# troyvvgroup/quemb

Hardware: AMD Instinct MI355X
Metric: fragment CCSD iters/sec (full BE sweep over synthetic n_occ=20 n_virt=200 fragments); corr-E error vs oracle in parity_max_abs_err_Eh / parity_n220_abs_err_Eh (higher is better)
Workload: dtype f64

## Files before the change

include/qemb_hip_ops.h:

```cpp
#ifndef QEMB_HIP_OPS_H
#define QEMB_HIP_OPS_H
#include "qemb_hip.h"
#ifdef __cplusplus
extern "C" {
#endif

#define QEMB_TIMER_LADDER 0
#define QEMB_TIMER_RINGS 1
#define QEMB_TIMER_ITER 2
#define QEMB_TIMER_AO2MO 3
#define QEMB_TIMER_SCF 4
#define QEMB_TIMER_GEMM_ANY 5
#define QEMB_TIMER_SCHMIDT 6
#define QEMB_TIMER_DF 7
int qemb_timer_begin(int slot);
int qemb_timer_end(int slot);
int qemb_timer_read(int slot, double* total_ms, int64_t* count);
int qemb_timer_reset(int slot);
int qemb_alloc_stats(long long* n_driver_allocs, long long* n_driver_frees, double* ms_in_driver_calls, double* gb_allocated, int reset);
int qemb_gemm_flop_count(double* flops, int reset);
int qemb_tape_cache_counters(int64_t* reused, int64_t* recorded, int reset);
int qemb_ctx_timer_read(int ctx, int slot, double* total_ms, int64_t* count, int reset);
int qemb_timer_live_events(int slot);

// ... 24 lines not shown
int qemb_op_dot(int64_t n, const double* x, const double* y, double* out_dev);
int qemb_op_absmax(int64_t n, const double* x, double* out_dev);
int qemb_op_gemv_rows(int64_t rows, int64_t cols, const double* T, int64_t ldt, const double* x, double* y,
                      double alpha, double beta);
int qemb_op_gemv_rows_batched(int64_t rows, int64_t cols, int64_t nbatch, const double* T, int64_t ldt, int64_t strideT,
                              const double* x, int64_t stridex, double* y, double alpha, double beta);
int qemb_op_contract_mid(int64_t outer, int64_t mid, int64_t inner, const double* T, const double* x,
                         double* Y, int64_t ldy, double alpha, double beta);
int qemb_op_unpack_s4(int64_t n, const double* s4, double* s1);
int qemb_op_pack_s4(int64_t n, const double* s1, double* s4);
int qemb_op_unpack_s8_to_s4(int64_t n, const double* s8, double* s4);
int qemb_op_mirror_lower(int64_t n, double* A, int64_t lda);
int qemb_op_k_from_pairs(int64_t n, const double* H, const double* D, double* K);
int qemb_op_jk_from_packed(int64_t n, const double* S4, const double* D, const double* Dp, double* Jp, double* K);
int qemb_op_pack_pm_cols(int64_t rows, int64_t v, const double* in, double* Op, int64_t ldp, double* Om, int64_t ldm);
int qemb_op_scatter_pm_rows(int64_t o, int64_t ncols, const double* Xp, const double* Xm, double* out);
int qemb_op_pack_w_pm(int64_t o, const double* W, double* Ap, int64_t lda_p, double* Am, int64_t lda_m);
int qemb_op_ladder_scatter_pm2(int64_t o, int64_t v, const double* Rp, int64_t ldp, const double* Rm, int64_t ldm, const double* Hp, const double* Hm,
                               int assign, double* t2);
int qemb_op_lincomb2(int64_t n, double a, const double* x, double b, const double* y, double beta, double* out);
int qemb_op_small_k_update(int64_t batch, int64_t M, int64_t N, int64_t K, double alpha, const double* A, int64_t sA, const double* B, int64_t sB, double* C, int64_t sC);
int qemb_op_ccsd_ph_layouts(int64_t o, int64_t v, const double* t2, const double* t1, double* T, double* Tp, double* S, double* Ut, double* Tpt, double* Th);
int qemb_op_ccsd_y_traces(int64_t o, int64_t v, const double* ZC, const double* ZB, double* Y);
int qemb_op_copy4_two(const int64_t dim[4], const double* in, const int64_t si[4], double* out, const int64_t so[4], double alpha, double beta, const double* base,
                      double* out2, const double* in2, double c2a, double c2b);
int qemb_op_scatter_pm_rows_add(int64_t o, int64_t ncols, const double* Xp, const double* Xm, double* out, const double* add);
int qemb_op_ccsd_y_traces_add(int64_t o, int64_t v, const double* ZC, const double* ZB, double* Y, const double* add);
int qemb_op_pack_w_pm_sum(int64_t o, const double* Wt, const double* X, const double* At, double* Ap, int64_t lda_p, double* Am, int64_t lda_m);
int qemb_op_ccsd_t1_small(int64_t o, int64_t v, const double* t1, const double* Lvv, const double* Loo, const double* Fov, double* t1n);
int qemb_op_ccsd_t1_assemble(int64_t o, int64_t v, const double* t1, const double* Lvv, const double* Loo, const double* Fov, const double* S, const double* Lph1,
                             const double* PA, int SA, int64_t strideA, const double* PB, int SB, int64_t strideB, double* t1n);
int qemb_op_gemv_rows_two(int64_t rows1, int64_t cols1, const double* T1, int64_t ld1, const double* x1, double* y1, double a1, double b1,
                          int64_t rows2, int64_t cols2, const double* T2, int64_t ld2, const double* x2, double* y2, double a2, double b2);
int qemb_op_ccsd_y_traces_slabs(int64_t o, int64_t v, const double* ZC, const double* ZB, double* Y, const double* add, int S, int64_t stride, double scale);
int qemb_op_gemv_rows2(int64_t rows, int64_t cols, const double* T1, int64_t ld1, const double* x1, const double* T2, int64_t ld2, const double* x2, double* y, double alpha, double beta);
int qemb_op_ccsd_finish_t2_rings(int64_t o, int64_t v, double* t2n, const double* U, const double* OV, const double* RS, const double* M, const double* eo, const double* ev, double* t1n);
int qemb_op_diis_push(int64_t n, const double* trial, const double* prev, double* e, double* xcopy, int m, const double* const* ys, int self, double* row_dev, double* row_host);
int qemb_op_ccsd_extrapolate_energy(int64_t o, int64_t v, int nterms, const double* coef, const double* const* xs, double* amp, const double* L, double* tau, double* e_host);
int qemb_op_gather_rows(int64_t nrows, int64_t len, const int64_t* idx_dev, const double* src, int64_t ld, double* dst);
int qemb_op_scale_rows(int64_t nrows, int64_t len, double* x, const double* s);
int qemb_op_pack_pair_rows(int64_t n, int64_t ncols, const double* in, double* out);
int qemb_op_unpack_tril_pair_rows(int64_t nr, int64_t n, const double* in, double* full);
int qemb_op_extract_pf(int64_t n, const double* Mp, int64_t p0, int64_t q0, int64_t r0, int64_t s0, int64_t sp, int64_t sq,
                       int64_t sr, int64_t ss, double* out);
int qemb_op_extract_pf_t(int64_t n, const double* T, int64_t x0, int64_t r0, int64_t s0, int64_t c0, int64_t sx, int64_t sr,
                         int64_t ss, int64_t sc, double* out);
// ... 40 lines not shown
```

quemb_amd/_lib.py:

```python

from __future__ import annotations

import ctypes as C
import os
from pathlib import Path

import numpy as np

_HERE = Path(__file__).resolve().parent
LIB_PATH = _HERE / "libqemb_hip.so"

c_dp = C.POINTER(C.c_double)
c_i64 = C.c_int64
c_vp = C.c_void_p


QEMB_ERR_ARG, QEMB_ERR_ALLOC, QEMB_ERR_DEVICE, QEMB_ERR_NOCONV, QEMB_ERR_NUMERIC, QEMB_ERR_UNSUPPORTED = -1, -2, -3, -4, -5, -6


class QembError(RuntimeError):

    def __init__(self, msg="", status=None):
        super().__init__(msg)
        self.status = status
# ... 58 lines not shown
    f("qemb_op_rdm2_add_nc", I, L, P, D, P)
    f("qemb_op_rdm2_symmetrize", I, L, P, P)
    f("qemb_op_rdm2_eri_dot", I, L, I, P, P, C.POINTER(D))
    f("qemb_op_absmax", I, L, P, P)
    f("qemb_op_gemv_rows", I, L, L, P, L, P, P, D, D)
    f("qemb_op_gemv_rows_batched", I, L, L, L, P, L, L, P, L, P, D, D)
    f("qemb_op_contract_mid", I, L, L, L, P, P, P, L, D, D)
    f("qemb_op_unpack_s4", I, L, P, P)
    f("qemb_op_pack_s4", I, L, P, P)
    f("qemb_op_unpack_s8_to_s4", I, L, P, P)
    f("qemb_op_unpack_tril_rows", I, L, L, P, P)
    f("qemb_op_pack_pair_rows", I, L, L, P, P)
    f("qemb_op_mirror_lower", I, L, P, L)
    f("qemb_op_k_from_pairs", I, L, P, P, P)
    f("qemb_op_jk_from_packed", I, L, P, P, P, P, P)
    f("qemb_op_pack_pm_cols", I, L, L, P, P, L, P, L)
    f("qemb_op_scatter_pm_rows", I, L, L, P, P, P)
    f("qemb_op_pack_w_pm", I, L, P, P, L, P, L)
    f("qemb_op_ladder_scatter_pm2", I, L, L, P, L, P, L, P, P, I, P)
    f("qemb_op_lincomb2", I, L, D, P, D, P, D, P)
    f("qemb_op_small_k_update", I, L, L, L, L, D, P, L, P, L, P, L)
    f("qemb_op_ccsd_ph_layouts", I, L, L, P, P, P, P, P, P, P, P)
    f("qemb_op_ccsd_y_traces", I, L, L, P, P, P)
    f("qemb_op_copy4_two", I, C.POINTER(L), P, C.POINTER(L), P, C.POINTER(L), D, D, P, P, P, D, D)
    f("qemb_op_scatter_pm_rows_add", I, L, L, P, P, P, P)
    f("qemb_op_ccsd_y_traces_add", I, L, L, P, P, P, P)
    f("qemb_op_pack_w_pm_sum", I, L, P, P, P, P, L, P, L)
    f("qemb_op_ccsd_t1_small", I, L, L, P, P, P, P, P)
    f("qemb_op_gemv_rows2", I, L, L, P, L, P, P, L, P, P, D, D)
    f("qemb_op_ccsd_t1_assemble", I, L, L, P, P, P, P, P, P, P, I, L, P, I, L, P)
    f("qemb_op_gemv_rows_two", I, L, L, P, L, P, P, D, D, L, L, P, L, P, P, D, D)
    f("qemb_op_ccsd_y_traces_slabs", I, L, L, P, P, P, P, I, L, D)
    f("qemb_op_ccsd_finish_t2_rings", I, L, L, P, P, P, P, P, P, P, P)
    f("qemb_op_diis_push", I, L, P, P, P, P, I, P, I, P, P)
    f("qemb_op_ccsd_extrapolate_energy", I, L, L, I, P, P, P, P, P, P)
    f("qemb_op_gather_rows", I, L, L, P, P, L, P)
    f("qemb_op_scale_rows", I, L, L, P, P)
    f("qemb_ctx_count", I, I)
    f("qemb_ctx_bind", I, I)
    f("qemb_ctx_partition", I, I)
    f("qemb_ctx_timer_read", I, I, I, C.POINTER(C.c_double), C.POINTER(c_i64), I)
    f("qemb_gemm_flop_count", I, C.POINTER(C.c_double), I)
    f("qemb_tape_cache_counters", I, C.POINTER(L), C.POINTER(L), I)
    f("qemb_alloc_stats", I, C.POINTER(C.c_longlong), C.POINTER(C.c_longlong), C.POINTER(C.c_double), C.POINTER(C.c_double), I)
    f("qemb_op_unpack_tril_pair_rows", I, L, L, P, P)
    f("qemb_op_extract_pf", I, L, P, L, L, L, L, L, L, L, L, P)
# ... 195 lines not shown
```

quemb_amd/csrc/api.cpp:

```cpp
#include <cstring>
#include <cstdlib>
#include <vector>
#include <execinfo.h>
#include <signal.h>
#include <unistd.h>
#include "../../include/qemb_hip_ops.h"
#include "dev_ops.h"
#include "ccsd.h"
#include "fragment.h"
#include "ao2mo.h"
#include "kdf.h"
#include "int3c.h"
#include "int4c.h"
#include <mutex>
#include <set>

using namespace qemb;
namespace qemb {
int dev_mfma_f64_peak(int iters, int blocks_per_cu, double* tflops);
int schmidt_eigh(const double* lmo, int N, int nmo, int nocc, const int64_t* frag, int n_f, double thr, double* TA_out,
                 int ld_out, int* n_b_out, int* sweeps_out);
int schmidt_subspace(const double* lmo, int N, int nmo, int nocc, const int64_t* frag, int n_f, double thr, double* TA_out,
                     int ld_out, int* n_b_out, int* sweeps_out);
int schmidt_svd(const double* rdm, int N, const int64_t* frag_in, int n_f, double thr, double* TA_out, int ld_out, int* n_b_out,
// ... 125 lines not shown
  tape_cache_counters(&a, &b, reset);
  if (reused) *reused = a;
  if (recorded) *recorded = b;
  return QEMB_OK;
}
int qemb_alloc_stats(long long* n, long long* nfree, double* ms, double* gb, int reset) { return dev_alloc_stats(n, nfree, ms, gb, reset); }
int qemb_ctx_timer_read(int ctx, int slot, double* total_ms, int64_t* count, int reset) { return dev_ctx_timer_read(ctx, slot, total_ms, count, reset); }
int qemb_op_k_from_pairs(int64_t n, const double* H, const double* D, double* K) { return dev_k_from_pairs(n, H, D, K); }
int qemb_op_jk_from_packed(int64_t n, const double* S4, const double* D, const double* Dp, double* Jp, double* K) { return dev_jk_from_packed(n, S4, D, Dp, Jp, K); }
int qemb_op_pack_pm_cols(int64_t rows, int64_t v, const double* in, double* Op, int64_t ldp, double* Om, int64_t ldm) { return dev_pack_pm_cols(rows, v, in, Op, ldp, Om, ldm); }
int qemb_op_scatter_pm_rows(int64_t o, int64_t ncols, const double* Xp, const double* Xm, double* out) { return dev_scatter_pm_rows(o, ncols, Xp, Xm, out); }
int qemb_op_pack_w_pm(int64_t o, const double* W, double* Ap, int64_t lda_p, double* Am, int64_t lda_m) { return dev_pack_w_pm(o, W, Ap, lda_p, Am, lda_m); }
int qemb_op_ladder_scatter_pm2(int64_t o, int64_t v, const double* Rp, int64_t ldp, const double* Rm, int64_t ldm, const double* Hp, const double* Hm,
                               int assign, double* t2) { return dev_ladder_scatter_pm2(o, v, Rp, ldp, Rm, ldm, Hp, Hm, assign, t2); }
int qemb_op_lincomb2(int64_t n, double a, const double* x, double b, const double* y, double beta, double* out) {
  const double c[2] = {a, b};
  const double* xs[2] = {x, y};
  return dev_lincomb(n, 2, c, xs, beta, out);
}
int qemb_op_mirror_lower(int64_t n, double* A, int64_t lda) { return dev_mirror_lower(n, A, lda); }
int qemb_op_small_k_update(int64_t batch, int64_t M, int64_t N, int64_t K, double alpha, const double* A, int64_t sA, const double* B, int64_t sB, double* C, int64_t sC) {
  return dev_small_k_update(batch, M, N, K, alpha, A, sA, B, sB, C, sC);
}
int qemb_op_ccsd_ph_layouts(int64_t o, int64_t v, const double* t2, const double* t1, double* T, double* Tp, double* S, double* Ut, double* Tpt, double* Th) {
  return dev_ccsd_ph_layouts(o, v, t2, t1, T, Tp, S, Ut, Tpt, Th);
}
int qemb_op_copy4_two(const int64_t dim[4], const double* in, const int64_t si[4], double* out, const int64_t so[4], double alpha, double beta, const double* base,
                      double* out2, const double* in2, double c2a, double c2b) {
  Copy4Desc c{};
  for (int k = 0; k < 4; ++k) { c.dim[k] = dim[k]; c.si[k] = si[k]; c.so[k] = so[k]; }
  c.in = in; c.out = out; c.alpha = alpha; c.beta = beta; c.base = base;
  c.out2 = out2; c.in2 = in2; c.c2a = c2a; c.c2b = c2b;
  return dev_copy4(c);
}
int qemb_op_scatter_pm_rows_add(int64_t o, int64_t ncols, const double* Xp, const double* Xm, double* out, const double* add) { return dev_scatter_pm_rows(o, ncols, Xp, Xm, out, add); }
int qemb_op_ccsd_y_traces_add(int64_t o, int64_t v, const double* ZC, const double* ZB, double* Y, const double* add) { return dev_ccsd_y_traces(o, v, ZC, ZB, Y, add); }
int qemb_op_pack_w_pm_sum(int64_t o, const double* Wt, const double* X, const double* At, double* Ap, int64_t lda_p, double* Am, int64_t lda_m) {
  return dev_pack_w_pm_sum(o, Wt, X, At, Ap, lda_p, Am, lda_m);
}
int qemb_op_ccsd_t1_small(int64_t o, int64_t v, const double* t1, const double* Lvv, const double* Loo, const double* Fov, double* t1n) { return dev_ccsd_t1_small(o, v, t1, Lvv, Loo, Fov, t1n); }
int qemb_op_ccsd_t1_assemble(int64_t o, int64_t v, const double* t1, const double* Lvv, const double* Loo, const double* Fov, const double* S, const double* Lph1,
                             const double* PA, int SA, int64_t strideA, const double* PB, int SB, int64_t strideB, double* t1n) {
  return dev_ccsd_t1_assemble(o, v, t1, Lvv, Loo, Fov, S, Lph1, PA, SA, strideA, PB, SB, strideB, t1n);
}
int qemb_op_gemv_rows_two(int64_t rows1, int64_t cols1, const double* T1, int64_t ld1, const double* x1, double* y1, double a1, double b1,
                          int64_t rows2, int64_t cols2, const double* T2, int64_t ld2, const double* x2, double* y2, double a2, double b2) {
// ... 697 lines not shown
```

quemb_amd/csrc/ccsd.cpp:

```cpp
#include "ccsd.h"
#include "ao2mo.h"
#include <algorithm>
#include <chrono>
#include <cmath>
#include <cstdio>
#include <cstdlib>
#include <cstring>
#include <string>

namespace qemb {

int mo_slab_ld(int n) { return (n >= 64 && n <= 1024) ? (n + 15) / 16 * 16 : n; }
int64_t mo_transform_work(int n) { return (int64_t)n * mo_slab_ld(n) * ((int64_t)n * (n + 1) / 2); }

static int mo_three_quarter_blocks(int n, int o, int nf, const double* T, int64_t slab, MoIntegrals& out, bool build_T34) {
  const int v = n - o;
  if (nf > 0 && build_T34) {
    QTRY(out.T34.alloc((int64_t)n * n * n * nf));
    QTRY(dev_extract_pf_t(n, T, 0, 0, 0, 0, n, n, n, nf, out.T34, slab));
  } else if (nf > 0) {
    QTRY(out.A1.alloc((int64_t)v * o * v * nf));
    QTRY(out.A2.alloc((int64_t)o * o * v * nf));
    QTRY(dev_extract_pf_t(n, T, o, 0, o, 0, v, o, v, nf, out.A1, slab));
    QTRY(dev_extract_pf_t(n, T, 0, 0, o, 0, o, o, v, nf, out.A2, slab));
// ... 370 lines not shown
  QTRY(dev_ccsd_t1_assemble(o, v, t1, Lvv_, Loo_, Fov_, S_, Lph1_, PA, spa.S, nov, PB, spb.S, nov, t1n));

  QTRY(gemm(o, oo * o, v, 1.0, t1, v, true, ovoo_cikl_, oo * o, false, 0.0, O1_, oo * o));
  QTRY(dev_pack_w_pm_sum(o, oooo_p_, Xw_, O1_, WAp_, lwp_, WAm_, lwm_));
  QTRY(apply_ladder(tau_, t2n, true, true));

  QTRY(gemm(oo * v, v, v, 1.0, t2, v, true, Lvv_, v, true, 0.0, U_, v));
  QTRY(gemm(o, o * vv, o, -1.0, Loo_, o, false, t2, o * vv, false, 1.0, U_, o * vv, 1, 0, 0, 0, cfg_wide));
  {
    const int64_t npo = o * (o + 1) / 2, nmo = o * (o - 1) / 2;
    int cfg, ks;
    SlabGemm sp, sm;
    pick_pair_gemm(npo, nov, cfg, ks, I_.ldp);
    QTRY(dev_region_begin());
    QTRY(gemm_slabs(npo, nov, I_.ldp, LTp_, I_.ldp, OVp_, I_.ldp, Xp_, nov, cfg, ks, sp));
    QTRY(dev_region_chain());
    if (nmo > 0) {
      pick_pair_gemm(nmo, nov, cfg, ks, I_.ldm);
      QTRY(gemm_slabs(nmo, nov, I_.ldm, LTm_, I_.ldm, OVm_, I_.ldm, Xm_, nov, cfg, ks, sm));
    }
    QTRY(dev_region_end());
    QTRY(dev_scatter_pm_rows(o, nov, Xp_, Xm_, X_, ovoo_ijka_, sp.S, sp.stride, sm.S, sm.stride));
  }
  QTRY(dev_region_begin());
  QTRY(perm4(U_, ZB_, o, v, v, o, 0, 3, 1, 2, 1.0, 1.0));
  QTRY(dev_region_chain());
  QTRY(gemm(oo * v, o, v, 1.0, I_.oovv, v, true, t1, v, true, 0.0, G2_, o, 1, 0, 0, 0, cfg_tall));
  QTRY(gemm(o, v * o, v, 1.0, t1, v, true, I_.ovvo, v * o, false, 1.0, G2_, v * o, o, 0, v * v * o, o * v * o, cfg_wide));
  QTRY(dev_region_end());
  QTRY(perm4(X_, G2_, o, o, v, o, 3, 1, 0, 2, 1.0, 1.0));
  QTRY(dev_small_k_update(oo, v, v, o, -1.0, X_, nov, t1, 0, U_, vv));
  TimerScope lap_RINGS(TIMER_RINGS);
  QTRY(dev_small_k_update(nov, v, o, o, -1.0, t1, 0, I_.ovoo, oo, ZB_, v * o));
  QTRY(perm4(W1_, ZB_, o, v, v, o, 3, 2, 0, 1, 1.0, 1.0, W1base_));
  const int64_t ring_tiles64 = ((nov + 63) / 64) * ((nov + 63) / 64) * dev_gemm_peers();
  static const bool ring96 = !(std::getenv("QEMB_RING96") && std::getenv("QEMB_RING96")[0] == '0');
  const bool mid_ring = ring96 && nov >= 1024 && nov < 2048 && dev_gemm_peers() == 1;
  const int cfg_ring = (nov >= 2048) ? 4 : mid_ring ? 37 : (nov >= 256 && ring_tiles64 >= 200) ? 1 : -1;
  auto ring = [&](double al, const double* A, const double* Bsym, double be, double* C) {
    return gemm(nov, nov, nov, al, A, nov, true, Bsym, nov, true, be, C, nov, 1, 0, 0, 0, cfg_ring, mid_ring ? 2 : 0);
  };
  QTRY(ring(0.25, W12_, Lovov_, 1.0, W1_));
  QTRY(dev_small_k_update(oo, v, v, o, -1.0, t1, 0, ovoo_kilc_, nov, ZC_, vv));
  {
    Copy4Desc c{};
    const int64_t d[4] = {o, o, v, v};
    const int perm[4] = {1, 2, 0, 3};
    int64_t od[4], ostr[4];
    for (int k = 0; k < 4; ++k) od[k] = d[perm[k]];
    ostr[3] = 1; ostr[2] = od[3]; ostr[1] = od[3] * od[2]; ostr[0] = od[3] * od[2] * od[1];
    c.in = ZC_; c.out = W2_; c.alpha = 1.0; c.beta = 1.0; c.base = W2base_;
    c.si[3] = 1; c.si[2] = d[3]; c.si[1] = d[3] * d[2]; c.si[0] = d[3] * d[2] * d[1];
    for (int k = 0; k < 4; ++k) { c.dim[k] = d[k]; c.so[perm[k]] = ostr[k]; }
    c.out2 = R_; c.in2 = W1_; c.c2a = 1.0; c.c2b = -0.5;
    QTRY(dev_copy4(c));
  }
  QTRY(ring(-0.5, W12b_, ovov_t_, 1.0, W2_));
  QTRY(dev_region_begin());
  QTRY(ring(1.0, W2_, Tp_, 0.0, W1_));
  QTRY(dev_region_chain());
  QTRY(ring(1.0, R_, S_, 0.0, W12_));
  QTRY(dev_region_end());
  QTRY(lap_RINGS.close());

  QTRY(dev_ccsd_finish_t2_rings(o, v, t2n, U_, OVoovv_, W12_, W1_, eo_, ev_, t1n));
  return 0;
}
// ... 295 lines not shown
```

quemb_amd/csrc/dev_ops.h:

```cpp
#pragma once
#include <cstddef>
#include <cstdint>
#include <string>
#include "../../include/qemb_hip_ops.h"

namespace qemb {

void set_error(const std::string& msg);
const char* last_error();



int dev_init(int device);
int dev_sync();
int dev_sync_device();
int dev_ctx_count(int n);
int dev_ctx_bind(int k);
int dev_ctx_partition(int parts);
int dev_alloc(void** p, size_t bytes);
int dev_free(void* p);
int dev_trim();
int dev_trim_all();
int dev_h2d(void* dst, const void* src_host, size_t bytes);
int dev_h2d_async(void* dst, const void* src, size_t bytes);
// ... 108 lines not shown

int dev_ladder_pack_vvvv(int64_t n, int64_t o, const double* M, double* Vp, int64_t ldp, double* Vm, int64_t ldm);
int dev_ladder_pack_tau(int64_t o, int64_t v, const double* tau, double* Tp, int64_t ldp, double* Tm, int64_t ldm);
int dev_pack_pm_cols(int64_t rows, int64_t v, const double* in, double* Op, int64_t ldp, double* Om, int64_t ldm);
int dev_scatter_pm_rows(int64_t o, int64_t ncols, const double* Xp, const double* Xm, double* out, const double* add = nullptr, int Sp = 1, int64_t strideP = 0,
                        int Sm = 1, int64_t strideM = 0);
int dev_ccsd_finish_t2(int64_t o, int64_t v, double* t2n, const double* U, const double* OV, const double* eo, const double* ev);
int dev_ccsd_finish_t2_rings(int64_t o, int64_t v, double* t2n, const double* U, const double* OV, const double* RS, const double* M, const double* eo, const double* ev, double* t1n);
int dev_ladder_scatter_pm(int64_t o, int64_t v, const double* Rp, int64_t ldp, const double* Rm, int64_t ldm, double* t2);
int dev_ladder_scatter_pm2(int64_t o, int64_t v, const double* Rp, int64_t ldp, const double* Rm, int64_t ldm, const double* Hp, const double* Hm,
                           int assign, double* t2, int Sp = 1, int64_t strideP = 0, int Sm = 1, int64_t strideM = 0, int64_t ldhp = 0, int64_t ldhm = 0);
int dev_pack_w_pm(int64_t o, const double* W, double* Ap, int64_t lda_p, double* Am, int64_t lda_m);
int dev_pack_w_pm_sum(int64_t o, const double* Wt, const double* X, const double* At, double* Ap, int64_t lda_p, double* Am, int64_t lda_m);
int dev_ccsd_t1_small(int64_t o, int64_t v, const double* t1, const double* Lvv, const double* Loo, const double* Fov, double* t1n);
int dev_ccsd_t1_assemble(int64_t o, int64_t v, const double* t1, const double* Lvv, const double* Loo, const double* Fov, const double* S, const double* Lph1,
                         const double* PA, int SA, int64_t strideA, const double* PB, int SB, int64_t strideB, double* t1n);
int dev_gemv_rows_two(int64_t rows1, int64_t cols1, const double* T1, int64_t ld1, const double* x1, double* y1, double a1, double b1,
                      int64_t rows2, int64_t cols2, const double* T2, int64_t ld2, const double* x2, double* y2, double a2, double b2);
int dev_gemv_rows2(int64_t rows, int64_t cols, const double* T1, int64_t ld1, const double* x1, const double* T2, int64_t ld2, const double* x2, double* y, double alpha, double beta);
int dev_foo_from_x(int64_t o, const double* X, double* F);
int dev_ccsd_ph_layouts(int64_t o, int64_t v, const double* t2, const double* t1, double* T, double* Tp, double* S, double* Ut, double* Tpt, double* Th);
int dev_small_k_update(int64_t batch, int64_t M, int64_t N, int64_t K, double alpha, const double* A, int64_t sA, const double* B, int64_t sB,
                       double* C, int64_t sC);
int dev_ccsd_y_traces(int64_t o, int64_t v, const double* ZC, const double* ZB, double* Y, const double* add = nullptr, int S = 1, int64_t stride = 0, double scale = 1.0);

inline int64_t dev_mp2_partial_count(int64_t o, int64_t v) {
  const int64_t nt = (v + 31) / 32, oo = o * o;
  return nt * (nt + 1) / 2 * (oo < 4096 ? oo : 4096);
}
int dev_mp2_amplitudes(int64_t o, int64_t v, const double* ovov, const double* eo, const double* ev, double* t2, double* G, double* partials, double* e_dev);

inline int rdm2_check_args(int kind, int64_t o, int64_t v, const double* t1, const double* t2, const double* out) {
  if (kind != QEMB_RDM2_CCSD && kind != QEMB_RDM2_MP2) { set_error("dev_rdm2_assemble: kind must be QEMB_RDM2_CCSD or QEMB_RDM2_MP2"); return QEMB_ERR_ARG; }
  if (o <= 0 || v < 0 || !out || (v > 0 && (!t2 || (kind == QEMB_RDM2_CCSD && !t1)))) { set_error("dev_rdm2_assemble: bad arguments"); return QEMB_ERR_ARG; }
  if (o + v > 32767) { set_error("dev_rdm2_assemble: n = " + std::to_string(o + v) + " is beyond any n^4 tensor"); return QEMB_ERR_ARG; }
  return 0;
}
int dev_rdm2_assemble(int kind, int64_t o, int64_t v, const double* t1, const double* t2, const double* dm1c, double* out);
inline int64_t rdm2_full_grid(int64_t m) { return m * m < 4096 ? m * m : 4096; }
inline int rdm2_check_full(int64_t m, const void* a, const void* b) {
  if (m <= 0 || m > 32767 || !a || !b) { set_error("rdm2 full-basis pass: bad arguments (N = " + std::to_string(m) + ")"); return QEMB_ERR_ARG; }
  return 0;
}
int dev_rdm2_add_nc(int64_t m, const double* g, double alpha, double* X);
int dev_rdm2_symmetrize(int64_t m, const double* g, double* X);
int dev_rdm2_eri_dot(int64_t m, int sym, const double* eri, const double* K, double* partials, double* out_dev);
// ... 86 lines not shown
```

quemb_amd/csrc/dev_ops_hip.hip:

```cpp
#include <hip/hip_runtime.h>
#include <chrono>
#include <atomic>
#include <algorithm>
#include <cstdint>
#include <cstdlib>
#include <cstring>
#include <map>
#include <thread>
#include <mutex>
#include <string>
#include <type_traits>
#include <vector>
#include "dev_ops.h"
#include "hip_common.h"
#include "grouped_launch.h"

namespace qemb {
static thread_local std::string g_err;
void set_error(const std::string& msg) { g_err = msg; }
const char* last_error() { return g_err.c_str(); }

struct TimerLap { hipEvent_t e0, e1; bool ended; };
struct TimerSlot { double total_ms = 0; int64_t count = 0; std::vector<TimerLap> pending; std::vector<std::pair<hipEvent_t, hipEvent_t>> spare; };
static constexpr size_t TIMER_MAX_PENDING = 64;
static constexpr int NPART = 2048;
struct DevCtx {
  hipStream_t stream = nullptr;
  std::atomic<bool> capturing{false};
  double* partials = nullptr;
  double* ws = nullptr;
  size_t ws_bytes = 0;
  double* gws = nullptr;
  size_t gws_bytes = 0;
  std::vector<std::pair<hipGraphNode_t, int>> marks;
  bool tape_capture = false, in_region = false;
  bool alloc_trace = false; unsigned long long alloc_hash = 0;
  size_t gws_bump = 0;
  TimerSlot timers[TIMER_NSLOTS];
// ... 1194 lines not shown
  }
}
__global__ void __launch_bounds__(256) small_k_update_mfma_kernel(int M, int N, int K, double alpha, const double* __restrict__ A, long long sA,
                                                                  const double* __restrict__ B, long long sB, double* __restrict__ C, long long sC) { small_k_update_mfma_kernel_body(make_uint3(blockIdx.x, blockIdx.y, blockIdx.z), make_uint3(gridDim.x, gridDim.y, gridDim.z), M, N, K, alpha, A, sA, B, sB, C, sC); }
int dev_small_k_update(int64_t batch, int64_t M, int64_t N, int64_t K, double alpha, const double* A, int64_t sA, const double* B, int64_t sB,
                       double* C, int64_t sC) {
  REQUIRE_INIT();
  if (batch <= 0 || M <= 0 || N <= 0 || K <= 0) return QEMB_OK;
  if (batch > 65535) { set_error("dev_small_k_update: batch too large"); return QEMB_ERR_ARG; }
  if (N >= 16 && M >= 16 && K <= 64 && M <= (1 << 20) && N <= (1 << 20)) {
    const long long items = ((M + 31) / 32) * ((N + 15) / 16);
    hipLaunchKernelGGL(small_k_update_mfma_kernel, dim3((unsigned)((items + 3) / 4), (unsigned)batch), dim3(256), 0, g_stream, (int)M, (int)N, (int)K, alpha,
                       A, (long long)sA, B, (long long)sB, C, (long long)sC);
    HIP_TRY(hipGetLastError());
    return QEMB_OK;
  }
  const long long tiles_m = (M + 31) / 32, tiles_n = (N + 31) / 32;
  hipLaunchKernelGGL(small_k_update_kernel, dim3((unsigned)(tiles_m * tiles_n), (unsigned)batch), dim3(256), 0, g_stream, (long long)M, (long long)N, (long long)K, alpha,
                     A, (long long)sA, B, (long long)sB, C, (long long)sC, (int)tiles_n);
  HIP_TRY(hipGetLastError());
  return QEMB_OK;
}

__device__ __forceinline__ double slab_sum(const double* __restrict__ p, int S, long long stride) {
  switch (S) {
    case 1: return p[0];
    case 2: { const double a = p[0], b = p[stride]; return a + b; }
    case 3: { const double a = p[0], b = p[stride], c = p[2 * stride]; return (a + b) + c; }
    case 4: { const double a = p[0], b = p[stride], c = p[2 * stride], d = p[3 * stride]; return ((a + b) + c) + d; }
    default: {
      double acc = 0.0;
      int sl = 0;
      for (; sl + 4 <= S; sl += 4) { const double a = p[sl * stride], b = p[(sl + 1) * stride], c = p[(sl + 2) * stride], d = p[(sl + 3) * stride]; acc = (((acc + a) + b) + c) + d; }
      for (; sl < S; ++sl) acc += p[sl * stride];
      return acc;
    }
  }
}
__device__ __forceinline__ void ccsd_y_traces_kernel_body(const uint3 BID, const uint3 GDIM, long long o, long long v, const double* __restrict__ ZC, const double* __restrict__ ZB,
                                                            double* __restrict__ Y, const double* __restrict__ add, int S, long long stride, double scale) {
  const long long idx = ((long long)BID.x * blockDim.x + threadIdx.x) >> 3;
  const int q = threadIdx.x & 7;
  const bool in = idx < v * v;
  const long long a = in ? idx / v : 0, c = in ? idx % v : 0;
  double s = 0.0;
  if (in) {
// ... 1736 lines not shown
  const long long np = n * (n + 1) / 2, n2 = n * n;
  for (long long r = blockIdx.x; r < rows; r += gridDim.x)
    for (long long kl = threadIdx.x; kl < n2; kl += blockDim.x) {
      const long long k = kl / n, l = kl - k * n;
      if (k >= l) packed[r * np + k * (k + 1) / 2 + l] = full[r * n2 + kl];
    }
}
int dev_pack_tril_rows(int64_t rows, int64_t n, const double* full, double* packed) {
  REQUIRE_INIT();
  if (rows <= 0) return QEMB_OK;
  hipLaunchKernelGGL(pack_tril_rows_kernel, dim3((unsigned)std::min<int64_t>(rows, 1 << 20)), dim3(256), 0, g_stream, (long long)rows, (long long)n, full, packed);
  HIP_TRY(hipGetLastError());
  return QEMB_OK;
}

static void register_groupable_kernels() {
  register_groupable<copy4_linear_kernel_body, 256, Copy4K>((const void*)copy4_linear_kernel);
  register_groupable<copy4_transpose_kernel_body, 256, Copy4K, int>((const void*)copy4_transpose_kernel);
  register_groupable<outer4_kernel_body, 256, Outer4K>((const void*)outer4_kernel);
  register_groupable<div_denom_kernel_body, 256, double*, long long, long long, long long, long long, const double*, const double*, const double*, const double*>((const void*)div_denom_kernel);
  register_groupable<ccsd_ph_layouts_kernel_body, 256, long long, long long, const double*, const double*, double*, double*, double*, double*, double*, double*, int>((const void*)ccsd_ph_layouts_kernel);
  register_groupable<small_k_update_kernel_body, 256, long long, long long, long long, double, const double*, long long, const double*, long long, double*, long long, int>((const void*)small_k_update_kernel);
  register_groupable<small_k_update_mfma_kernel_body, 256, int, int, int, double, const double*, long long, const double*, long long, double*, long long>((const void*)small_k_update_mfma_kernel);
  register_groupable<ccsd_y_traces_kernel_body, 256, long long, long long, const double*, const double*, double*, const double*, int, long long, double>((const void*)ccsd_y_traces_kernel);
  register_groupable<lincomb_kernel_body, 256, long long, LincombK, double, double*>((const void*)lincomb_kernel);
  register_groupable<ladder_pack_tau_kernel_body, 256, long long, long long, const double*, double*, long long, double*, long long>((const void*)ladder_pack_tau_kernel);
  register_groupable<scatter_pm_rows_kernel_body, 256, long long, long long, const double*, const double*, double*, const double*, int, long long, int, long long>((const void*)scatter_pm_rows_kernel);
  register_groupable<ccsd_finish_t2_kernel_body, 256, long long, long long, double*, const double*, const double*, const double*, const double*>((const void*)ccsd_finish_t2_kernel);
  register_groupable<ladder_scatter_pm_kernel_body, 256, long long, long long, const double*, long long, const double*, long long, double*, const double*, const double*, int, int, long long, int, long long, long long, long long>((const void*)ladder_scatter_pm_kernel);
  register_groupable<pack_w_pm_kernel_body, 256, long long, const double*, double*, long long, double*, long long>((const void*)pack_w_pm_kernel);
  register_groupable<pack_w_pm_sum_kernel_body, 256, long long, const double*, const double*, const double*, double*, long long, double*, long long>((const void*)pack_w_pm_sum_kernel);
  register_groupable<foo_from_x_kernel_body, 256, long long, const double*, double*>((const void*)foo_from_x_kernel);
  register_groupable<gemv_rows2_kernel_body, 256, long long, long long, const double*, long long, const double*, const double*, long long, const double*, double*, double, double>((const void*)gemv_rows2_kernel);
  register_groupable<ccsd_t1_small_kernel_body, 256, int, int, const double*, const double*, const double*, const double*, double*>((const void*)ccsd_t1_small_kernel);
  register_groupable<ccsd_t1_assemble_kernel_body, 256, int, int, const double*, const double*, const double*, const double*, const double*, const double*, const double*, int, long long, const double*, int, long long, double*>((const void*)ccsd_t1_assemble_kernel);
  register_groupable<gemv_rows_two_kernel_body, 256, long long, long long, const double*, long long, const double*, double*, double, double, long long, long long, const double*, long long, const double*, double*, double, double>((const void*)gemv_rows_two_kernel);
  register_groupable<ccsd_finish_t2_rings_kernel_body, 256, long long, long long, double*, const double*, const double*, const double*, const double*, const double*, const double*, double*>((const void*)ccsd_finish_t2_rings_kernel);
  register_groupable<gemv_rows_kernel_body, 256, long long, long long, const double*, long long, const double*, double*, double, double>((const void*)gemv_rows_kernel);
  register_groupable<contract_mid_stage1_body, 256, long long, long long, int, const double*, const double*, double*>((const void*)contract_mid_stage1);
  register_groupable<contract_mid_stage2_body, 256, long long, long long, int, const double*, double*, long long, double, double>((const void*)contract_mid_stage2);
  register_groupable<unpack_tril_rows_kernel_body, 256, long long, long long, const double*, double*>((const void*)unpack_tril_rows_kernel);
  register_groupable<unpack_tril_tiled_kernel_body, 256, long long, long long, const double*, double*, int, long long, long long>((const void*)unpack_tril_tiled_kernel);
  register_groupable<fill_kernel_body, 1024, double*, long long, double>((const void*)fill_kernel);
}

}
// ... 1 lines not shown
```

Measured before the change: 57.40.

## Fuse ZB/ZC small-k updates with permute-accumulate into tail consume kernels

Adds two new kernels that each fold a t1·ovoo small-K contraction (done with f64 MFMA) into the permuting copy that consumes ZB or ZC. One writes U and W1, the other writes W2 and R directly from tiles held in shared memory or registers, replacing several separate small_k_update and perm4 passes over o·v·v·o arrays. The aim is to remove intermediate global memory round-trips and kernel launches in the ring tail. The path is on by default behind an environment toggle. It adds custom tiling with cache-line alignment shifts, which makes boundary-handling bugs more likely.

After: 57.67, median of 6. No clear change (+0.5%).

```diff
diff --git a/include/qemb_hip_ops.h b/include/qemb_hip_ops.h
--- a/include/qemb_hip_ops.h
+++ b/include/qemb_hip_ops.h
@@ -70,6 +70,8 @@
 int qemb_op_small_k_update(int64_t batch, int64_t M, int64_t N, int64_t K, double alpha, const double* A, int64_t sA, const double* B, int64_t sB, double* C, int64_t sC);
 int qemb_op_ccsd_ph_layouts(int64_t o, int64_t v, const double* t2, const double* t1, double* T, double* Tp, double* S, double* Ut, double* Tpt, double* Th);
 int qemb_op_ccsd_y_traces(int64_t o, int64_t v, const double* ZC, const double* ZB, double* Y);
+int qemb_op_ccsd_zb_consume(int64_t o, int64_t v, const double* ZB, const double* t1, const double* ovoo, double* U, const double* W1base, double* W1);
+int qemb_op_ccsd_zc_consume(int64_t o, int64_t v, const double* ZC, const double* t1, const double* ovoo_kilc, const double* W2base, const double* W1, double* W2, double* R);
 int qemb_op_copy4_two(const int64_t dim[4], const double* in, const int64_t si[4], double* out, const int64_t so[4], double alpha, double beta, const double* base,
                       double* out2, const double* in2, double c2a, double c2b);
 int qemb_op_scatter_pm_rows_add(int64_t o, int64_t ncols, const double* Xp, const double* Xm, double* out, const double* add);
diff --git a/quemb_amd/_lib.py b/quemb_amd/_lib.py
--- a/quemb_amd/_lib.py
+++ b/quemb_amd/_lib.py
@@ -104,6 +104,8 @@
     f("qemb_op_small_k_update", I, L, L, L, L, D, P, L, P, L, P, L)
     f("qemb_op_ccsd_ph_layouts", I, L, L, P, P, P, P, P, P, P, P)
     f("qemb_op_ccsd_y_traces", I, L, L, P, P, P)
+    f("qemb_op_ccsd_zb_consume", I, L, L, P, P, P, P, P, P)
+    f("qemb_op_ccsd_zc_consume", I, L, L, P, P, P, P, P, P, P)
     f("qemb_op_copy4_two", I, C.POINTER(L), P, C.POINTER(L), P, C.POINTER(L), D, D, P, P, P, D, D)
     f("qemb_op_scatter_pm_rows_add", I, L, L, P, P, P, P)
     f("qemb_op_ccsd_y_traces_add", I, L, L, P, P, P, P)
diff --git a/quemb_amd/csrc/api.cpp b/quemb_amd/csrc/api.cpp
--- a/quemb_amd/csrc/api.cpp
+++ b/quemb_amd/csrc/api.cpp
@@ -171,6 +171,12 @@
 int qemb_op_small_k_update(int64_t batch, int64_t M, int64_t N, int64_t K, double alpha, const double* A, int64_t sA, const double* B, int64_t sB, double* C, int64_t sC) {
   return dev_small_k_update(batch, M, N, K, alpha, A, sA, B, sB, C, sC);
 }
+int qemb_op_ccsd_zb_consume(int64_t o, int64_t v, const double* ZB, const double* t1, const double* ovoo, double* U, const double* W1base, double* W1) {
+  return dev_ccsd_zb_consume(o, v, ZB, t1, ovoo, U, W1base, W1);
+}
+int qemb_op_ccsd_zc_consume(int64_t o, int64_t v, const double* ZC, const double* t1, const double* ovoo_kilc, const double* W2base, const double* W1, double* W2, double* R) {
+  return dev_ccsd_zc_consume(o, v, ZC, t1, ovoo_kilc, W2base, W1, W2, R);
+}
 int qemb_op_ccsd_ph_layouts(int64_t o, int64_t v, const double* t2, const double* t1, double* T, double* Tp, double* S, double* Ut, double* Tpt, double* Th) {
   return dev_ccsd_ph_layouts(o, v, t2, t1, T, Tp, S, Ut, Tpt, Th);
 }
diff --git a/quemb_amd/csrc/ccsd.cpp b/quemb_amd/csrc/ccsd.cpp
--- a/quemb_amd/csrc/ccsd.cpp
+++ b/quemb_amd/csrc/ccsd.cpp
@@ -416,8 +416,10 @@
     QTRY(dev_region_end());
     QTRY(dev_scatter_pm_rows(o, nov, Xp_, Xm_, X_, ovoo_ijka_, sp.S, sp.stride, sm.S, sm.stride));
   }
+  static const bool tail_fused = !(std::getenv("QEMB_TAIL_FUSED") && std::getenv("QEMB_TAIL_FUSED")[0] == '0');
   QTRY(dev_region_begin());
-  QTRY(perm4(U_, ZB_, o, v, v, o, 0, 3, 1, 2, 1.0, 1.0));
+  if (tail_fused) QTRY(dev_ccsd_zb_consume(o, v, ZB_, t1, I_.ovoo, U_, W1base_, W1_));
+  else QTRY(perm4(U_, ZB_, o, v, v, o, 0, 3, 1, 2, 1.0, 1.0));
   QTRY(dev_region_chain());
   QTRY(gemm(oo * v, o, v, 1.0, I_.oovv, v, true, t1, v, true, 0.0, G2_, o, 1, 0, 0, 0, cfg_tall));
   QTRY(gemm(o, v * o, v, 1.0, t1, v, true, I_.ovvo, v * o, false, 1.0, G2_, v * o, o, 0, v * v * o, o * v * o, cfg_wide));
@@ -425,8 +427,10 @@
   QTRY(perm4(X_, G2_, o, o, v, o, 3, 1, 0, 2, 1.0, 1.0));
   QTRY(dev_small_k_update(oo, v, v, o, -1.0, X_, nov, t1, 0, U_, vv));
   TimerScope lap_RINGS(TIMER_RINGS);
-  QTRY(dev_small_k_update(nov, v, o, o, -1.0, t1, 0, I_.ovoo, oo, ZB_, v * o));
-  QTRY(perm4(W1_, ZB_, o, v, v, o, 3, 2, 0, 1, 1.0, 1.0, W1base_));
+  if (!tail_fused) {
+    QTRY(dev_small_k_update(nov, v, o, o, -1.0, t1, 0, I_.ovoo, oo, ZB_, v * o));
+    QTRY(perm4(W1_, ZB_, o, v, v, o, 3, 2, 0, 1, 1.0, 1.0, W1base_));
+  }
   const int64_t ring_tiles64 = ((nov + 63) / 64) * ((nov + 63) / 64) * dev_gemm_peers();
   static const bool ring96 = !(std::getenv("QEMB_RING96") && std::getenv("QEMB_RING96")[0] == '0');
   const bool mid_ring = ring96 && nov >= 1024 && nov < 2048 && dev_gemm_peers() == 1;
@@ -435,8 +439,10 @@
     return gemm(nov, nov, nov, al, A, nov, true, Bsym, nov, true, be, C, nov, 1, 0, 0, 0, cfg_ring, mid_ring ? 2 : 0);
   };
   QTRY(ring(0.25, W12_, Lovov_, 1.0, W1_));
-  QTRY(dev_small_k_update(oo, v, v, o, -1.0, t1, 0, ovoo_kilc_, nov, ZC_, vv));
-  {
+  if (!tail_fused) QTRY(dev_small_k_update(oo, v, v, o, -1.0, t1, 0, ovoo_kilc_, nov, ZC_, vv));
+  if (tail_fused) {
+    QTRY(dev_ccsd_zc_consume(o, v, ZC_, t1, ovoo_kilc_, W2base_, W1_, W2_, R_));
+  } else {
     Copy4Desc c{};
     const int64_t d[4] = {o, o, v, v};
     const int perm[4] = {1, 2, 0, 3};
diff --git a/quemb_amd/csrc/dev_ops.h b/quemb_amd/csrc/dev_ops.h
--- a/quemb_amd/csrc/dev_ops.h
+++ b/quemb_amd/csrc/dev_ops.h
@@ -154,6 +154,8 @@
 int dev_ccsd_ph_layouts(int64_t o, int64_t v, const double* t2, const double* t1, double* T, double* Tp, double* S, double* Ut, double* Tpt, double* Th);
 int dev_small_k_update(int64_t batch, int64_t M, int64_t N, int64_t K, double alpha, const double* A, int64_t sA, const double* B, int64_t sB,
                        double* C, int64_t sC);
+int dev_ccsd_zb_consume(int64_t o, int64_t v, const double* ZB, const double* t1, const double* ovoo, double* U, const double* W1base, double* W1);
+int dev_ccsd_zc_consume(int64_t o, int64_t v, const double* ZC, const double* t1, const double* ovoo_kilc, const double* W2base, const double* W1, double* W2, double* R);
 int dev_ccsd_y_traces(int64_t o, int64_t v, const double* ZC, const double* ZB, double* Y, const double* add = nullptr, int S = 1, int64_t stride = 0, double scale = 1.0);
 
 inline int64_t dev_mp2_partial_count(int64_t o, int64_t v) {
diff --git a/quemb_amd/csrc/dev_ops_hip.hip b/quemb_amd/csrc/dev_ops_hip.hip
--- a/quemb_amd/csrc/dev_ops_hip.hip
+++ b/quemb_amd/csrc/dev_ops_hip.hip
@@ -14,6 +14,7 @@
 #include "dev_ops.h"
 #include "hip_common.h"
 #include "grouped_launch.h"
+#include "tail_tiling.h"
 
 namespace qemb {
 static thread_local std::string g_err;
@@ -1254,6 +1255,168 @@
   return QEMB_OK;
 }
 
+__device__ __forceinline__ void ccsd_zb_consume_kernel_body(const uint3 BID, const uint3 GDIM, int o, int v, const double* __restrict__ ZB, const double* __restrict__ t1,
+                                                              const double* __restrict__ ovoo, double* __restrict__ U, const double* __restrict__ W1base, double* __restrict__ W1) {
+  __shared__ double tile[ZB_T * ZB_SC];
+  const uint3 LB = xcd_logical_block(BID, GDIM);
+  const long long k = LB.y;
+  const ZbGrid g = zb_grid(o, v);
+  const ZbTile t = zb_tile(g, LB.x, o, v, k);
+  const int lane = threadIdx.x & 63, wave = threadIdx.x >> 6;
+  {
+    const unsigned run = (unsigned)(ZB_T * t.icw), magic = zb_div_magic(t.icw > 0 ? t.icw : 1);
+#pragma unroll
+    for (int q = 0; q < ZB_T / 4; ++q) {
+      const int cc = wave + 4 * q, cg = t.c0 + cc;
+      const bool cin = cg >= 0 && cg < v;
+      const double* __restrict__ src = ZB + (((long long)k * v + (cin ? cg : 0)) * v + t.a0) * o + t.i0;
+#pragma unroll
+      for (int m = 0; m < (ZB_T * ZB_IC + 63) / 64; ++m) {
+        const unsigned e = (unsigned)lane + 64u * m;
+        if (e < run) {
+          const int a = zb_div(e, magic), i = (int)e - a * t.icw;
+          tile[cc * ZB_SC + a * ZB_SI + i] = (cin && t.a0 + a < v) ? src[(long long)a * o + i] : 0.0;
+        }
+      }
+    }
+  }
+  __syncthreads();
+  {
+    const int a = threadIdx.x & 15, c = threadIdx.x >> 4;
+    const int ag = t.a0 + a, cg = t.c0 + c;
+    if (ag < v && cg >= 0 && cg < v) {
+      const long long vv = (long long)v * v;
+      double* __restrict__ up = U + (((long long)k * o + t.i0) * v + cg) * v + ag;
+      const double* __restrict__ lp = tile + c * ZB_SC + a * ZB_SI;
+      int i = 0;
+      for (; i + 4 <= t.icw; i += 4) {
+        const double u0 = up[(long long)i * vv], u1 = up[(long long)(i + 1) * vv], u2 = up[(long long)(i + 2) * vv], u3 = up[(long long)(i + 3) * vv];
+        up[(long long)i * vv] = lp[i] + u0; up[(long long)(i + 1) * vv] = lp[i + 1] + u1;
+        up[(long long)(i + 2) * vv] = lp[i + 2] + u2; up[(long long)(i + 3) * vv] = lp[i + 3] + u3;
+      }
+      for (; i < t.icw; ++i) up[(long long)i * vv] = lp[i] + up[(long long)i * vv];
+    }
+  }
+  __syncthreads();
+  {
+    const int fr = lane & 15, fk = lane >> 4;
+    const bool ain = t.a0 + fr < v;
+    for (int cc = wave; cc < ZB_T; cc += 4) {
+      const int cg = t.c0 + cc;
+      if (cg < 0 || cg >= v) continue;
+      const double* __restrict__ Bz = ovoo + ((long long)k * v + cg) * o * o;
+      for (int n0 = 0; n0 < t.icw; n0 += 16) {
+        const int il = n0 + fr;
+        const bool iin = il < t.icw;
+        d4v acc = {0.0, 0.0, 0.0, 0.0};
+        for (int k0 = 0; k0 < o; k0 += 4) {
+          const int l = k0 + fk;
+          const bool lin = l < o;
+          const double b = (lin && iin) ? Bz[(long long)l * o + t.i0 + il] : 0.0;
+          const double a = (lin && ain) ? t1[(long long)l * v + t.a0 + fr] : 0.0;
+          acc = __builtin_amdgcn_mfma_f64_16x16x4f64(a, b, acc, 0, 0, 0);
+        }
+        if (iin) {
+#pragma unroll
+          for (int r = 0; r < 4; ++r) tile[cc * ZB_SC + (fk + 4 * r) * ZB_SI + il] -= acc[r];
+        }
+      }
+    }
+  }
+  __syncthreads();
+  {
+    const int c = threadIdx.x & 15, a = threadIdx.x >> 4;
+    const int ag = t.a0 + a, cg = t.c0 + c;
+    if (ag < v && cg >= 0 && cg < v) {
+      const long long si = (long long)v * o * v;
+      const long long off = (((long long)t.i0 * v + ag) * o + k) * v + cg;
+      const double* __restrict__ bp = W1base + off;
+      double* __restrict__ wp = W1 + off;
+      const double* __restrict__ lp = tile + c * ZB_SC + a * ZB_SI;
+      int i = 0;
+      for (; i + 4 <= t.icw; i += 4) {
+        const double b0 = bp[(long long)i * si], b1 = bp[(long long)(i + 1) * si], b2 = bp[(long long)(i + 2) * si], b3 = bp[(long long)(i + 3) * si];
+        wp[(long long)i * si] = lp[i] + b0; wp[(long long)(i + 1) * si] = lp[i + 1] + b1;
+        wp[(long long)(i + 2) * si] = lp[i + 2] + b2; wp[(long long)(i + 3) * si] = lp[i + 3] + b3;
+      }
+      for (; i < t.icw; ++i) wp[(long long)i * si] = lp[i] + bp[(long long)i * si];
+    }
+  }
+}
+__global__ void __launch_bounds__(256) ccsd_zb_consume_kernel(int o, int v, const double* __restrict__ ZB, const double* __restrict__ t1, const double* __restrict__ ovoo,
+                                                               double* __restrict__ U, const double* __restrict__ W1base, double* __restrict__ W1) { ccsd_zb_consume_kernel_body(make_uint3(blockIdx.x, blockIdx.y, blockIdx.z), make_uint3(gridDim.x, gridDim.y, gridDim.z), o, v, ZB, t1, ovoo, U, W1base, W1); }
+int dev_ccsd_zb_consume(int64_t o, int64_t v, const double* ZB, const double* t1, const double* ovoo, double* U, const double* W1base, double* W1) {
+  REQUIRE_INIT();
+  if (o <= 0 || v <= 0) return QEMB_OK;
+  if (!ZB || !t1 || !ovoo || !U || !W1base || !W1) { set_error("dev_ccsd_zb_consume: null pointer"); return QEMB_ERR_ARG; }
+  if (o > 65535 || v > (1 << 20)) { set_error("dev_ccsd_zb_consume: extent too large"); return QEMB_ERR_ARG; }
+  const ZbGrid g = zb_grid(o, v);
+  const long long gx = (long long)g.tiles_c * g.tiles_a * g.nch;
+  if (gx > 0x7fffffffLL) { set_error("dev_ccsd_zb_consume: too many tiles"); return QEMB_ERR_ARG; }
+  hipLaunchKernelGGL(ccsd_zb_consume_kernel, dim3((unsigned)gx, (unsigned)o), dim3(256), 0, g_stream, (int)o, (int)v, ZB, t1, ovoo, U, W1base, W1);
+  HIP_TRY(hipGetLastError());
+  return QEMB_OK;
+}
+
+__device__ __forceinline__ void ccsd_zc_consume_kernel_body(const uint3 BID, const uint3 GDIM, int o, int v, const double* __restrict__ ZC, const double* __restrict__ t1,
+                                                              const double* __restrict__ ovoo_kilc, const double* __restrict__ W2base, const double* __restrict__ W1,
+                                                              double* __restrict__ W2, double* __restrict__ R) {
+  const int lane = threadIdx.x & 63, fr = lane & 15, fk = lane >> 4;
+  const uint3 LB = xcd_logical_block(BID, GDIM);
+  const long long z = LB.y, k = z / o, i = z - k * o;
+  const int item = (int)LB.x * 4 + (int)(threadIdx.x >> 6);
+  if (item >= zc_row_strips(v) * zc_col_tiles(o, v, k)) return;
+  const ZcItem it = zc_item(item, o, v, k);
+  const int m0 = it.m0, col = it.col0 + fr;
+  const bool cin = col >= 0 && col < v;
+  const double* __restrict__ Cz = ZC + z * v * v;
+  const double* __restrict__ Bz = ovoo_kilc + z * o * v;
+  const long long orow = (long long)o * v, obase = (i * v * o + k) * v + col;
+  const int ra = m0 + fr, rb = ra + 16;
+  double c0[4], c1[4], p0[4], p1[4], w0[4], w1[4];
+#pragma unroll
+  for (int r = 0; r < 4; ++r) {
+    const int ma = m0 + fk + 4 * r, mb = ma + 16;
+    const bool ina = cin && ma < v, inb = cin && mb < v;
+    c0[r] = ina ? Cz[(long long)ma * v + col] : 0.0;
+    c1[r] = inb ? Cz[(long long)mb * v + col] : 0.0;
+    p0[r] = ina ? W2base[obase + ma * orow] : 0.0;
+    p1[r] = inb ? W2base[obase + mb * orow] : 0.0;
+    w0[r] = ina ? W1[obase + ma * orow] : 0.0;
+    w1[r] = inb ? W1[obase + mb * orow] : 0.0;
+  }
+  d4v acc0 = {0.0, 0.0, 0.0, 0.0}, acc1 = {0.0, 0.0, 0.0, 0.0};
+  for (int k0 = 0; k0 < o; k0 += 4) {
+    const int l = k0 + fk;
+    const bool lin = l < o;
+    const double b = (lin && cin) ? Bz[(long long)l * v + col] : 0.0;
+    const double a0 = (lin && ra < v) ? t1[(long long)l * v + ra] : 0.0;
+    const double a1 = (lin && rb < v) ? t1[(long long)l * v + rb] : 0.0;
+    acc0 = __builtin_amdgcn_mfma_f64_16x16x4f64(a0, b, acc0, 0, 0, 0);
+    acc1 = __builtin_amdgcn_mfma_f64_16x16x4f64(a1, b, acc1, 0, 0, 0);
+  }
+  if (cin) {
+#pragma unroll
+    for (int r = 0; r < 4; ++r) {
+      const int ma = m0 + fk + 4 * r, mb = ma + 16;
+      if (ma < v) { const double w = (c0[r] - acc0[r]) + p0[r]; W2[obase + ma * orow] = w; R[obase + ma * orow] = w0[r] - 0.5 * w; }
+      if (mb < v) { const double w = (c1[r] - acc1[r]) + p1[r]; W2[obase + mb * orow] = w; R[obase + mb * orow] = w1[r] - 0.5 * w; }
+    }
+  }
+}
+__global__ void __launch_bounds__(256) ccsd_zc_consume_kernel(int o, int v, const double* __restrict__ ZC, const double* __restrict__ t1, const double* __restrict__ ovoo_kilc,
+                                                               const double* __restrict__ W2base, const double* __restrict__ W1, double* __restrict__ W2, double* __restrict__ R) { ccsd_zc_consume_kernel_body(make_uint3(blockIdx.x, blockIdx.y, blockIdx.z), make_uint3(gridDim.x, gridDim.y, gridDim.z), o, v, ZC, t1, ovoo_kilc, W2base, W1, W2, R); }
+int dev_ccsd_zc_consume(int64_t o, int64_t v, const double* ZC, const double* t1, const double* ovoo_kilc, const double* W2base, const double* W1, double* W2, double* R) {
+  REQUIRE_INIT();
+  if (o <= 0 || v <= 0) return QEMB_OK;
+  if (!ZC || !t1 || !ovoo_kilc || !W2base || !W1 || !W2 || !R) { set_error("dev_ccsd_zc_consume: null pointer"); return QEMB_ERR_ARG; }
+  if (o * o > 65535 || v > (1 << 20)) { set_error("dev_ccsd_zc_consume: extent too large"); return QEMB_ERR_ARG; }
+  const long long items = zc_items_max(v);
+  hipLaunchKernelGGL(ccsd_zc_consume_kernel, dim3((unsigned)((items + 3) / 4), (unsigned)(o * o)), dim3(256), 0, g_stream, (int)o, (int)v, ZC, t1, ovoo_kilc, W2base, W1, W2, R);
+  HIP_TRY(hipGetLastError());
+  return QEMB_OK;
+}
+
 __device__ __forceinline__ double slab_sum(const double* __restrict__ p, int S, long long stride) {
   switch (S) {
     case 1: return p[0];
@@ -3036,6 +3199,8 @@
   register_groupable<ccsd_ph_layouts_kernel_body, 256, long long, long long, const double*, const double*, double*, double*, double*, double*, double*, double*, int>((const void*)ccsd_ph_layouts_kernel);
   register_groupable<small_k_update_kernel_body, 256, long long, long long, long long, double, const double*, long long, const double*, long long, double*, long long, int>((const void*)small_k_update_kernel);
   register_groupable<small_k_update_mfma_kernel_body, 256, int, int, int, double, const double*, long long, const double*, long long, double*, long long>((const void*)small_k_update_mfma_kernel);
+  register_groupable<ccsd_zb_consume_kernel_body, 256, int, int, const double*, const double*, const double*, double*, const double*, double*>((const void*)ccsd_zb_consume_kernel);
+  register_groupable<ccsd_zc_consume_kernel_body, 256, int, int, const double*, const double*, const double*, const double*, const double*, double*, double*>((const void*)ccsd_zc_consume_kernel);
   register_groupable<ccsd_y_traces_kernel_body, 256, long long, long long, const double*, const double*, double*, const double*, int, long long, double>((const void*)ccsd_y_traces_kernel);
   register_groupable<lincomb_kernel_body, 256, long long, LincombK, double, double*>((const void*)lincomb_kernel);
   register_groupable<ladder_pack_tau_kernel_body, 256, long long, long long, const double*, double*, long long, double*, long long>((const void*)ladder_pack_tau_kernel);
diff --git a/quemb_amd/csrc/tail_ops_hostcheck.cpp b/quemb_amd/csrc/tail_ops_hostcheck.cpp
--- /dev/null
+++ b/quemb_amd/csrc/tail_ops_hostcheck.cpp
@@ -0,0 +1,35 @@
+#ifdef QEMB_HOSTCHECK
+#include "dev_ops.h"
+
+namespace qemb {
+
+int dev_ccsd_zb_consume(int64_t o, int64_t v, const double* ZB, const double* t1, const double* ovoo, double* U, const double* W1base, double* W1) {
+  if (o <= 0 || v <= 0) return 0;
+  if (!ZB || !t1 || !ovoo || !U || !W1base || !W1) { set_error("dev_ccsd_zb_consume: null pointer"); return QEMB_ERR_ARG; }
+  for (int64_t k = 0; k < o; ++k) for (int64_t c = 0; c < v; ++c) for (int64_t a = 0; a < v; ++a) for (int64_t i = 0; i < o; ++i) {
+    const double z = ZB[((k * v + c) * v + a) * o + i];
+    double s = 0.0;
+    for (int64_t l = 0; l < o; ++l) s += t1[l * v + a] * ovoo[((k * v + c) * o + l) * o + i];
+    U[((k * o + i) * v + c) * v + a] += z;
+    const int64_t off = ((i * v + a) * o + k) * v + c;
+    W1[off] = W1base[off] + (z - s);
+  }
+  return 0;
+}
+
+int dev_ccsd_zc_consume(int64_t o, int64_t v, const double* ZC, const double* t1, const double* ovoo_kilc, const double* W2base, const double* W1, double* W2, double* R) {
+  if (o <= 0 || v <= 0) return 0;
+  if (!ZC || !t1 || !ovoo_kilc || !W2base || !W1 || !W2 || !R) { set_error("dev_ccsd_zc_consume: null pointer"); return QEMB_ERR_ARG; }
+  for (int64_t k = 0; k < o; ++k) for (int64_t i = 0; i < o; ++i) for (int64_t a = 0; a < v; ++a) for (int64_t c = 0; c < v; ++c) {
+    double s = 0.0;
+    for (int64_t l = 0; l < o; ++l) s += t1[l * v + a] * ovoo_kilc[((k * o + i) * o + l) * v + c];
+    const int64_t off = ((i * v + a) * o + k) * v + c;
+    const double w = W2base[off] + (ZC[((k * o + i) * v + a) * v + c] - s);
+    W2[off] = w;
+    R[off] = W1[off] - 0.5 * w;
+  }
+  return 0;
+}
+
+}
+#endif
diff --git a/quemb_amd/csrc/tail_tiling.h b/quemb_amd/csrc/tail_tiling.h
--- /dev/null
+++ b/quemb_amd/csrc/tail_tiling.h
@@ -0,0 +1,51 @@
+#pragma once
+#if defined(__HIPCC__) || defined(__CUDACC__)
+#define QEMB_TT_HD __host__ __device__ __forceinline__
+#else
+#define QEMB_TT_HD inline
+#endif
+
+namespace qemb {
+constexpr int ZB_T = 16;
+constexpr int ZB_IC = 24;
+constexpr int ZB_SI = ZB_IC + 1;
+constexpr int ZB_SC = ZB_T * ZB_SI + 1;
+struct ZbGrid { int tiles_c, tiles_a, nch, icw; };
+struct ZbTile { int c0, a0, i0, icw; };
+
+QEMB_TT_HD int tail_line_shift(long long o, long long v, long long k) { return ((o * v) % 16 == 0) ? (int)((k * v) % 16) : 0; }
+
+QEMB_TT_HD ZbGrid zb_grid(long long o, long long v) {
+  ZbGrid g;
+  g.tiles_c = (int)((v + 15 + ZB_T - 1) / ZB_T);
+  g.tiles_a = (int)((v + ZB_T - 1) / ZB_T);
+  g.nch = (int)((o + ZB_IC - 1) / ZB_IC);
+  g.icw = (int)((o + g.nch - 1) / g.nch);
+  return g;
+}
+QEMB_TT_HD ZbTile zb_tile(const ZbGrid& g, unsigned x, long long o, long long v, long long k) {
+  ZbTile t;
+  const int ta = (int)(x % (unsigned)g.tiles_a), rest = (int)(x / (unsigned)g.tiles_a);
+  const int ich = rest % g.nch, tc = rest / g.nch;
+  t.c0 = tc * ZB_T - tail_line_shift(o, v, k);
+  t.a0 = ta * ZB_T;
+  t.i0 = ich * g.icw;
+  const long long left = o - t.i0;
+  t.icw = (int)(left < g.icw ? (left > 0 ? left : 0) : g.icw);
+  return t;
+}
+QEMB_TT_HD unsigned zb_div_magic(int icw) { return (65536u + (unsigned)icw - 1u) / (unsigned)icw; }
+QEMB_TT_HD int zb_div(unsigned e, unsigned magic) { return (int)((e * magic) >> 16); }
+
+struct ZcItem { int m0, col0; };
+QEMB_TT_HD int zc_col_tiles(long long o, long long v, long long k) { return (int)((v + tail_line_shift(o, v, k) + 15) / 16); }
+QEMB_TT_HD int zc_row_strips(long long v) { return (int)((v + 31) / 32); }
+QEMB_TT_HD long long zc_items_max(long long v) { return (long long)zc_row_strips(v) * ((v + 15 + 15) / 16); }
+QEMB_TT_HD ZcItem zc_item(int item, long long o, long long v, long long k) {
+  const int nt = zc_col_tiles(o, v, k);
+  ZcItem it;
+  it.m0 = (item / nt) * 32;
+  it.col0 = (item % nt) * 16 - tail_line_shift(o, v, k);
+  return it;
+}
+}
```
